# IQTLabs/WITW

Measured on AMD Instinct MI355X. Metric: image-pairs/sec (embedding+similarity), higher is better.
Workload: dtype f32

## Files before the change

witw_amd/csrc/conv3x3.hip:

```cpp
#include "common.h"
#include <stdlib.h>
#include <algorithm>

namespace {

constexpr int TW_WIDE = 64;

__device__ const f32x4 g_zero_f4[1] = {{0.f, 0.f, 0.f, 0.f}};

struct ConvArgs {
    const float* x;
    const float* wpk;
    const float* bias;
    const float* dropmask;
    const float* post_scale;
    const float* post_shift;
    float lrelu;
    unsigned char* pool_code;
    const float* gate;
    float* y;
    int B, H, W, Cin, Cout;
    int Ho, Wo;
    int tiles_x, tiles_y;
    int n_tiles, sp_total, sp_per_xcd, xcd_map;
    int circ, relu, out_nchw;
    int force_nw;
    int force_geo;
    int dil_h;
    int tap_base;
    int ksplit, kc_per_split;
    size_t split_stride;
    int s2d, s2d_h, s2d_w, valid_h, valid_w;
    int wino;
    const float* wpk_wino;
#ifdef WITW_STAMPS
    unsigned long long* stamps;
#endif
};

template <int NW, bool POOL>
__device__ __forceinline__ void conv_wino_h2(const ConvArgs& p, f32x4* smem) {
    constexpr int TH = NW, TW = 64, IW = TW + 2, IH = TH + 2;
    constexpr int NTHREADS = 64 * NW;
    constexpr int WTN = 64;
    constexpr int IN_F4 = 2 * IH * IW;
    constexpr int W_F4 = 12 * 2 * WTN;
    constexpr int STAGE_F4 = IN_F4 + W_F4;
    constexpr int NIN = (IN_F4 + NTHREADS - 1) / NTHREADS;
    constexpr int NWT = W_F4 / NTHREADS;
    static_assert(NWT * NTHREADS == W_F4, "the filter slab splits evenly over the workgroup");

    const int tid = threadIdx.x;
    const int lane = tid & 63;
    const int wave = tid >> 6;
    const int l31 = lane & 31;
    const int hq = lane >> 5;

    int ntile, sp;
    if (p.xcd_map) {
        const int g = blockIdx.x >> 3;
        ntile = g % p.n_tiles;
        sp = (blockIdx.x & 7) * p.sp_per_xcd + g / p.n_tiles;
        if (sp >= p.sp_total) return;
    } else {
        ntile = blockIdx.x / p.sp_total;
        sp = blockIdx.x - ntile * p.sp_total;
    }
    const int tiles_img = p.tiles_x * p.tiles_y;
    const int b = sp / tiles_img;
    sp -= b * tiles_img;
    const int ty = sp / p.tiles_x;
    const int tx = sp - ty * p.tiles_x;
    const int oy0 = ty * TH;
    const int ox0 = tx * TW;
    const int n0 = ntile * WTN;
    const int nkc = p.Cin >> 3;

    constexpr unsigned OOR = 0x80000000u;
    const size_t img_floats = (size_t)p.H * p.W * p.Cin;
    __amdgpu_buffer_rsrc_t in_rs = __builtin_amdgcn_make_buffer_rsrc((void*)(p.x + (size_t)b * img_floats), 0,
                                                                     (unsigned)(img_floats * 4), 0x00020000);
    __amdgpu_buffer_rsrc_t w_rs = __builtin_amdgcn_make_buffer_rsrc(
        (void*)(reinterpret_cast<const f32x4*>(p.wpk_wino) + (size_t)ntile * nkc * W_F4), 0, (unsigned)nkc * W_F4 * 16u, 0x00020000);
    unsigned gin[NIN];
#pragma unroll
    for (int i = 0; i < NIN; ++i) {
        const int s = tid + i * NTHREADS;
        const int pix = s >> 1, q = s & 1;
        const int r = pix / IW, c = pix - r * IW;
        const int gr = oy0 - 1 + r;
        int gc = ox0 - 1 + c;
        bool ok = (s < IN_F4) && gr >= 0 && gr < p.H;
        if (p.circ) {
            gc %= p.W;
            if (gc < 0) gc += p.W;
        } else {
            ok = ok && gc >= 0 && gc < p.W;
        }
        gin[i] = ok ? (unsigned)((((size_t)gr * p.W + gc) * p.Cin + q * 4) * 4) : OOR;
    }
    const unsigned gwoff = (unsigned)tid * 16u;
    f32x4 rin[NIN], rw[NWT];
    auto load_stage = [&](int kc) {
#pragma unroll
        for (int i = 0; i < NIN; ++i)
            rin[i] = __builtin_bit_cast(f32x4, __builtin_amdgcn_raw_buffer_load_b128(in_rs, gin[i], (unsigned)kc * 32u, 0));
        const unsigned wbase = (unsigned)kc * W_F4 * 16u;
#pragma unroll
        for (int i = 0; i < NWT; ++i)
            rw[i] = __builtin_bit_cast(f32x4, __builtin_amdgcn_raw_buffer_load_b128(w_rs, gwoff, wbase + (unsigned)i * (NTHREADS * 16u), 0));
    };
    auto store_stage = [&](int buf) {
        f32x4* in_s = smem + buf * STAGE_F4;
        f32x4* w_s = in_s + IN_F4;
#pragma unroll
        for (int i = 0; i < NIN; ++i) {
            const int s = tid + i * NTHREADS;
            f32x4* dst = (NIN * NTHREADS == IN_F4 || s < IN_F4) ? in_s + (s & 1) * (IH * IW) + (s >> 1) : smem + 2 * STAGE_F4;
            *dst = rin[i];
        }
#pragma unroll
        for (int i = 0; i < NWT; ++i) w_s[tid + i * NTHREADS] = rw[i];
    };

    const int wm = wave >> 1, wn = wave & 1;
    const int abase = hq * (IH * IW) + 2 * wm * IW + l31;
    const int wbase = hq * WTN + wn * 32 + l31;
    f32x16 acc[4][2];
#pragma unroll
    for (int t = 0; t < 4; ++t)
#pragma unroll
        for (int ct = 0; ct < 2; ++ct)
#pragma unroll
            for (int r = 0; r < 16; ++r) acc[t][ct][r] = 0.f;

    f32x4 fa[2][4], fb[2][4];
    auto read_a = [&](int set, const f32x4* in_s, int s) {
#pragma unroll
        for (int i = 0; i < 4; ++i) fa[set][i] = in_s[abase + i * IW + 32 * (s & 1) + (s >> 1)];
    };
    auto read_b = [&](int set, const f32x4* w_s, int kw) {
#pragma unroll
        for (int t = 0; t < 4; ++t) fb[set][t] = w_s[(kw * 4 + t) * 2 * WTN + wbase];
    };
    auto transform = [&](int set) {
#pragma unroll
        for (int j = 0; j < 4; ++j) {
            const float d0 = fa[set][0][j], d1 = fa[set][1][j], d2 = fa[set][2][j], d3 = fa[set][3][j];
            fa[set][0][j] = d0 - d2;
            fa[set][1][j] = d1 + d2;
            fa[set][2][j] = d2 - d1;
            fa[set][3][j] = d1 - d3;
        }
    };
    auto mfma_step = [&](int set, int bset, int ct) {
#pragma unroll
        for (int j = 0; j < 4; ++j)
#pragma unroll
            for (int t = 0; t < 4; ++t)
                acc[t][ct] = __builtin_amdgcn_mfma_f32_32x32x2f32(fa[set][t][j], fb[bset][t][j], acc[t][ct], 0, 0, 0);
    };

    load_stage(0);
    store_stage(0);
    __syncthreads();
    read_a(0, smem, 0);
    read_b(0, smem + IN_F4, 0);
    transform(0);

#define SG_STEP(NR, MASK, NX)                                           \
    do {                                                                \
        _Pragma("unroll") for (int i_ = 0; i_ < (NR); ++i_) {           \
            __builtin_amdgcn_sched_group_barrier(0x008, 1, 0);          \
            __builtin_amdgcn_sched_group_barrier(0x100, 1, 0);          \
        }                                                               \
        _Pragma("unroll") for (int i_ = 0; i_ < (NX); ++i_) {           \
            __builtin_amdgcn_sched_group_barrier(0x008, 1, 0);          \
            __builtin_amdgcn_sched_group_barrier(MASK, 1, 0);           \
        }                                                               \
        _Pragma("unroll") for (int i_ = 0; i_ < 16 - (NR) - (NX); ++i_) \
            __builtin_amdgcn_sched_group_barrier(0x008, 1, 0);          \
    } while (0)
    static_assert(16 - 4 - (NIN + NWT) >= 0, "step too short to hide the staging instructions");

    for (int kc = 0; kc < nkc; ++kc) {
        const int cur = kc & 1;
        const int kn = (kc + 1 < nkc) ? kc + 1 : kc;
        const f32x4* in_s = smem + cur * STAGE_F4;
        const f32x4* w_s = in_s + IN_F4;
        const f32x4* in_n = smem + (cur ^ 1) * STAGE_F4;
        read_a(1, in_s, 1);
        load_stage(kn);
        mfma_step(0, 0, 0);
        transform(1);
        SG_STEP(4, 0x020, NIN + NWT);
        read_a(0, in_s, 2);
        read_b(1, w_s, 1);
        mfma_step(1, 0, 1);
        transform(0);
        SG_STEP(8, 0x020, 0);
        read_a(1, in_s, 3);
        read_b(0, w_s, 2);
        mfma_step(0, 1, 0);
        transform(1);
        SG_STEP(8, 0x020, 0);
        read_a(0, in_s, 4);
        store_stage(cur ^ 1);
        mfma_step(1, 1, 1);
        transform(0);
        SG_STEP(4, 0x200, NIN + NWT);
        read_a(1, in_s, 5);
        mfma_step(0, 0, 0);
        transform(1);
        SG_STEP(4, 0x020, 0);
        __syncthreads();
        read_a(0, in_n, 0);
        read_b(1, in_n + IN_F4, 0);
        mfma_step(1, 0, 1);
        transform(0);
        SG_STEP(8, 0x020, 0);
#pragma unroll
        for (int t = 0; t < 4; ++t) fb[0][t] = fb[1][t];
    }
#undef SG_STEP

    f32x16 yv[2][2];
#pragma unroll
    for (int ct = 0; ct < 2; ++ct)
#pragma unroll
        for (int r = 0; r < 16; ++r) {
            const float m0 = acc[0][ct][r], m1 = acc[1][ct][r], m2 = acc[2][ct][r], m3 = acc[3][ct][r];
            yv[0][ct][r] = (m0 + m1) + m2;
            yv[1][ct][r] = (m1 - m2) - m3;
        }
    const int nb = n0 + wn * 32;
    const int nch = nb + l31;
    const float bv = p.bias[nch];
    const float dm = (p.dropmask != nullptr && nch < p.Cout) ? p.dropmask[(size_t)b * p.Cout + nch] : 1.f;
    const int act = p.relu;
    auto fin = [&](float v) {
        v = (v + bv) * dm;
        if (act == 1) v = fmaxf(v, 0.f);
        else if (act == 2) v = v > 0.f ? v : v * p.lrelu;
        return v;
    };
    const int Hy = POOL ? (p.Ho >> 1) : p.Ho;
    const int Wy = POOL ? (p.Wo >> 1) : p.Wo;
    float* slab = reinterpret_cast<float*>(smem) + wave * (32 * 32);
    const int prow = lane >> 3, pc4 = (lane & 7) * 4;
    if constexpr (!POOL) {
#pragma unroll
        for (int k = 0; k < 2; ++k)
#pragma unroll
            for (int ct = 0; ct < 2; ++ct) {
#pragma unroll
                for (int r = 0; r < 16; ++r) slab[((r & 3) + 8 * (r >> 2) + 4 * hq) * 32 + l31] = fin(yv[k][ct][r]);
                const int yy = oy0 + 2 * wm + k;
#pragma unroll
                for (int g = 0; g < 4; ++g) {
                    const int m = g * 8 + prow;
                    const f32x4 v = *reinterpret_cast<const f32x4*>(slab + m * 32 + pc4);
                    const int xx = ox0 + 32 * ct + m;
                    if (yy < Hy && xx < Wy && nb + pc4 < p.Cout)
                        __builtin_nontemporal_store(v, reinterpret_cast<f32x4*>(p.y + (((size_t)b * Hy + yy) * Wy + xx) * p.Cout + nb + pc4));
                }
            }
    } else {
        const int yy = (oy0 + 2 * wm) >> 1;
#pragma unroll
        for (int ct = 0; ct < 2; ++ct)
#pragma unroll
            for (int g = 0; g < 4; ++g)
#pragma unroll
                for (int e = 0; e < 2; ++e) {
                    const int r = 4 * g + 2 * e;
                    const float a00 = yv[0][ct][r], a01 = yv[0][ct][r + 1], a10 = yv[1][ct][r], a11 = yv[1][ct][r + 1];
                    const float m = fmaxf(fmaxf(a00, a01), fmaxf(a10, a11));
                    const int pc = 16 * ct + 4 * g + 2 * hq + e;
                    slab[pc * 32 + l31] = fin(m);
                    const int xx = (ox0 >> 1) + pc;
                    if (p.pool_code != nullptr && yy < Hy && xx < Wy && nch < p.Cout) {
                        const int code = (a00 == m) ? 0 : (a01 == m) ? 1 : (a10 == m) ? 2 : 3;
                        p.pool_code[(((size_t)b * Hy + yy) * Wy + xx) * p.Cout + nch] = (unsigned char)code;
                    }
                }
#pragma unroll
        for (int g = 0; g < 4; ++g) {
            const int pc = g * 8 + prow;
            const f32x4 v = *reinterpret_cast<const f32x4*>(slab + pc * 32 + pc4);
            const int xx = (ox0 >> 1) + pc;
            if (yy < Hy && xx < Wy && nb + pc4 < p.Cout)
                __builtin_nontemporal_store(v, reinterpret_cast<f32x4*>(p.y + (((size_t)b * Hy + yy) * Wy + xx) * p.Cout + nb + pc4));
        }
    }
}

template <int TN, int SH, bool POOL, int NW, int GEO, int TAPS = 9>
__global__ __launch_bounds__(64 * NW) void conv3x3_nhwc_f32_kernel(ConvArgs p) {
    static_assert(TAPS == 9 || TAPS == 4, "3x3 window or a 2x2 sub-window");
    constexpr bool NARROW = GEO == 1;
    constexpr bool DIL = GEO == 2;
    static_assert(!DIL || (TN == 128 && NW == 8 && SH == 1 && TAPS == 9 && !POOL), "the dilated form exists for the 8-wave 128-channel tile");
    constexpr int TH = NARROW ? 4 * NW : NW;
    constexpr int TW = NARROW ? 16 : 64;
    constexpr int IW = TW + 2;
    constexpr int NTHREADS = 64 * NW;
    constexpr int IH = (TH - 1) * SH + 3;
    constexpr int IN_F4 = 2 * IH * IW;
    constexpr int W_F4 = TAPS * 2 * TN;
    constexpr int STAGE_F4 = IN_F4 + W_F4;
    constexpr int NIN = (IN_F4 + NTHREADS - 1) / NTHREADS;
    constexpr int NWT = (W_F4 + NTHREADS - 1) / NTHREADS;
    constexpr int WGM = (TN == 128) ? NW / 2 : NW;
    constexpr int WM = (2 * NW) / WGM;
    constexpr int WN = 2;

    constexpr bool WINO = SH == 1 && TAPS == 9 && GEO == 0 && (TN == 128 || POOL);
    constexpr int WINO_F4 = WINO ? 2 * (2 * (NW + 2) * IW + 12 * 2 * 64) + 1 : 0;
    constexpr int DIRECT_F4 = (2 * STAGE_F4 + 1 > NW * 512) ? 2 * STAGE_F4 + 1 : NW * 512;
    constexpr int SMEM_F4 = DIRECT_F4 > WINO_F4 ? DIRECT_F4 : WINO_F4;
    __shared__ f32x4 smem[SMEM_F4];
    static_assert(SMEM_F4 * 16 >= NW * 32 * 64 * 4, "the buffer must hold one epilogue slab per wave");
    if constexpr (WINO) {
        if (p.wino) {
            conv_wino_h2<NW, POOL>(p, smem);
            return;
        }
    }

    const int tid = threadIdx.x;
    const int lane = tid & 63;
    const int wave = tid >> 6;
    const int l31 = lane & 31;
    const int hq = lane >> 5;

    int ntile, sp;
    if (p.xcd_map) {
        const int g = blockIdx.x >> 3;
        ntile = g % p.n_tiles;
        sp = (blockIdx.x & 7) * p.sp_per_xcd + g / p.n_tiles;
        if (sp >= p.sp_total) return;
    } else {
        ntile = blockIdx.x / p.sp_total;
        sp = blockIdx.x - ntile * p.sp_total;
    }
    const int tiles_img = p.tiles_x * p.tiles_y;
    const int b = sp / tiles_img;
    sp -= b * tiles_img;
    const int ty = sp / p.tiles_x;
    const int tx = sp - ty * p.tiles_x;
    const int oy0 = ty * TH;
    const int ox0 = tx * TW;
    const int n0 = ntile * TN;
    int nkc = p.Cin >> 3;
    int kc_lo = 0;
    if constexpr (TAPS == 4) {
        if (p.ksplit > 1) {
            kc_lo = (int)blockIdx.y * p.kc_per_split;
            nkc = min(nkc - kc_lo, p.kc_per_split);
        }
    }

    constexpr unsigned OOR = 0x80000000u;
    const int Hp = p.dil_h ? (p.H - 1) / 2 + 1 : p.H;
    const size_t img_floats = (size_t)Hp * p.W * p.Cin;
    __amdgpu_buffer_rsrc_t in_rs = __builtin_amdgcn_make_buffer_rsrc(
        (void*)(p.x + (size_t)b * img_floats + (size_t)kc_lo * 8), 0, (unsigned)(img_floats * 4) - (unsigned)kc_lo * 32u, 0x00020000);
    const unsigned wtile_bytes = (unsigned)nkc * W_F4 * 16u;
    __amdgpu_buffer_rsrc_t w_rs = __builtin_amdgcn_make_buffer_rsrc(
        (void*)(reinterpret_cast<const f32x4*>(p.wpk) + ((size_t)ntile * (p.Cin >> 3) + kc_lo) * W_F4), 0, wtile_bytes, 0x00020000);
    unsigned gin[NIN];
#pragma unroll
    for (int i = 0; i < NIN; ++i) {
        const int s = tid + i * NTHREADS;
        const int pix = s >> 1, q = s & 1;
        const int r = pix / IW, c = pix - r * IW;
        const int gr = oy0 * SH - 1 + r;
        int gc = ox0 - 1 + c;
        bool ok = (s < IN_F4) && gr >= 0 && gr < p.H;
        int grp = gr;
        if (p.dil_h) {
            ok = ok && (gr & 1) == 0;
            grp = gr >> 1;
        }
        if (p.circ) {
            gc %= p.W;
            if (gc < 0) gc += p.W;
        } else {
            ok = ok && gc >= 0 && gc < p.W;
        }
        gin[i] = ok ? (unsigned)((((size_t)grp * p.W + gc) * p.Cin + q * 4) * 4) : OOR;
    }
    const unsigned gwoff = (unsigned)tid * 16u;

    f32x4 rin[NIN], rw[NWT];
    auto load_stage = [&](int kc) {
#pragma unroll
        for (int i = 0; i < NIN; ++i)
            rin[i] = __builtin_bit_cast(f32x4, __builtin_amdgcn_raw_buffer_load_b128(in_rs, gin[i], (unsigned)kc * 32u, 0));
        const unsigned wbase = (unsigned)kc * W_F4 * 16u;
#pragma unroll
        for (int i = 0; i < NWT; ++i)
            rw[i] = __builtin_bit_cast(f32x4, __builtin_amdgcn_raw_buffer_load_b128(w_rs, gwoff, wbase + (unsigned)i * (NTHREADS * 16u), 0));
    };
    auto store_stage = [&](int buf) {
        f32x4* in_s = smem + buf * STAGE_F4;
        f32x4* w_s = in_s + IN_F4;
#pragma unroll
        for (int i = 0; i < NIN; ++i) {
            const int s = tid + i * NTHREADS;
            f32x4* dst = (NIN * NTHREADS == IN_F4 || s < IN_F4) ? in_s + (s & 1) * (IH * IW) + (s >> 1) : smem + 2 * STAGE_F4;
            *dst = rin[i];
        }
#pragma unroll
        for (int i = 0; i < NWT; ++i) {
            const int s = tid + i * NTHREADS;
            f32x4* dst = (NWT * NTHREADS == W_F4 || s < W_F4) ? w_s + s : smem + 2 * STAGE_F4;
            *dst = rw[i];
        }
    };

    const int wm = (TN == 128) ? (wave >> 1) : wave;
    const int wn = (TN == 128) ? (wave & 1) : 0;
    int trow[WM], tcol[WM];
#pragma unroll
    for (int mt = 0; mt < WM; ++mt) {
        if (NARROW) {
            trow[mt] = 2 * ((TN == 128 ? 4 : 2) * wm + mt);
            tcol[mt] = 0;
        } else if (TN == 128) {
            trow[mt] = 2 * wm + (mt >> 1);
            tcol[mt] = 32 * (mt & 1);
        } else {
            trow[mt] = 2 * (wm >> 1) + mt;
            tcol[mt] = 32 * (wm & 1);
        }
    }
    auto m_row = [](int m) { return NARROW ? (m >> 4) : 0; };
    auto m_col = [](int m) { return NARROW ? (m & 15) : m; };
    int abase[WM];
#pragma unroll
    for (int mt = 0; mt < WM; ++mt)
        abase[mt] = hq * (IH * IW) + (trow[mt] + m_row(l31)) * SH * IW + tcol[mt] + m_col(l31) + (TAPS == 4 ? p.tap_base * (IW + 1) : 0);
    const int wbase = hq * TN + wn * 64 + l31;

    f32x16 acc[WM][WN];
#pragma unroll
    for (int mt = 0; mt < WM; ++mt)
#pragma unroll
        for (int nt = 0; nt < WN; ++nt)
#pragma unroll
            for (int r = 0; r < 16; ++r) acc[mt][nt][r] = 0.f;

    f32x4 fa[2][WM], fb[2][WN];
    auto live = [](int mt, int tap) { return !DIL || ((((mt >> 1) + tap / 3) & 1) == 1); };
    auto read_frags = [&](int set, const f32x4* in_s, const f32x4* w_s, int tap) {
        const int kh = (TAPS == 4) ? (tap >> 1) : tap / 3, kw = (TAPS == 4) ? (tap & 1) : tap - kh * 3;
#pragma unroll
        for (int mt = 0; mt < WM; ++mt)
            if (live(mt, tap)) fa[set][mt] = in_s[abase[mt] + kh * IW + kw];
#pragma unroll
        for (int nt = 0; nt < WN; ++nt) fb[set][nt] = w_s[tap * 2 * TN + wbase + nt * 32];
    };
    auto mfma_tap = [&](int set, int tap) {
#pragma unroll
        for (int j = 0; j < 4; ++j)
#pragma unroll
            for (int mt = 0; mt < WM; ++mt)
                if (live(mt, tap)) {
#pragma unroll
                    for (int nt = 0; nt < WN; ++nt)
                        acc[mt][nt] =
                            __builtin_amdgcn_mfma_f32_32x32x2f32(fa[set][mt][j], fb[set][nt][j], acc[mt][nt], 0, 0, 0);
                }
    };

#ifdef WITW_STAMPS
    unsigned long long t_stamp[6];
    int n_stamp = 0;
#define STAMP() do { if (n_stamp < 6) t_stamp[n_stamp++] = __builtin_amdgcn_s_memtime(); } while (0)
    const unsigned long long r_stamp0 = __builtin_amdgcn_s_memrealtime();
#else
#define STAMP() do { } while (0)
#endif
    STAMP();
    load_stage(0);
    store_stage(0);
    __syncthreads();
    read_frags(0, smem, smem + IN_F4, 0);
    STAMP();

    constexpr int MPT = 4 * (DIL ? WM / 2 : WM) * WN;
    constexpr int RPT = (DIL ? WM / 2 : WM) + WN;
#define SG_PLAIN_TAP()                                                  \
    do {                                                                \
        _Pragma("unroll") for (int i_ = 0; i_ < RPT; ++i_) {            \
            __builtin_amdgcn_sched_group_barrier(0x008, 2, 0);          \
            __builtin_amdgcn_sched_group_barrier(0x100, 1, 0);          \
        }                                                               \
        _Pragma("unroll") for (int i_ = 0; i_ < MPT - 2 * RPT; ++i_)    \
            __builtin_amdgcn_sched_group_barrier(0x008, 1, 0);          \
    } while (0)
#define SG_HEAVY_TAP(MASK, NX)                                          \
    do {                                                                \
        _Pragma("unroll") for (int i_ = 0; i_ < RPT; ++i_) {            \
            __builtin_amdgcn_sched_group_barrier(0x008, 1, 0);          \
            __builtin_amdgcn_sched_group_barrier(0x100, 1, 0);          \
        }                                                               \
        _Pragma("unroll") for (int i_ = 0; i_ < (NX); ++i_) {           \
            __builtin_amdgcn_sched_group_barrier(0x008, 1, 0);          \
            __builtin_amdgcn_sched_group_barrier(MASK, 1, 0);           \
        }                                                               \
        _Pragma("unroll") for (int i_ = 0; i_ < MPT - RPT - (NX); ++i_) \
            __builtin_amdgcn_sched_group_barrier(0x008, 1, 0);          \
    } while (0)
    static_assert(MPT - RPT - (NIN + NWT) >= 0, "tap too short to hide the staging instructions");

    if constexpr (TAPS == 4) {
        for (int kc = 0; kc < nkc; ++kc) {
            const int cur = kc & 1;
            const int kn = (kc + 1 < nkc) ? kc + 1 : kc;
            const f32x4* in_s = smem + cur * STAGE_F4;
            const f32x4* w_s = in_s + IN_F4;
            const f32x4* in_n = smem + (cur ^ 1) * STAGE_F4;
            read_frags(1, in_s, w_s, 1);
            load_stage(kn);
            mfma_tap(0, 0);
            SG_HEAVY_TAP(0x020, NIN + NWT);
            read_frags(0, in_s, w_s, 2);
            mfma_tap(1, 1);
            SG_PLAIN_TAP();
            read_frags(1, in_s, w_s, 3);
            store_stage(cur ^ 1);
            mfma_tap(0, 2);
            SG_HEAVY_TAP(0x200, NIN + NWT);
            __syncthreads();
            read_frags(0, in_n, in_n + IN_F4, 0);
            mfma_tap(1, 3);
            SG_PLAIN_TAP();
        }
    } else {
        for (int kc = 0; kc < nkc; ++kc) {
            const int cur = kc & 1;
            const int kn = (kc + 1 < nkc) ? kc + 1 : kc;
            const f32x4* in_s = smem + cur * STAGE_F4;
            const f32x4* w_s = in_s + IN_F4;
            const f32x4* in_n = smem + (cur ^ 1) * STAGE_F4;
            read_frags(1, in_s, w_s, 1);
#ifndef WITW_DIAG_NOSTAGE
            load_stage(kn);
#endif
            mfma_tap(0, 0);
            SG_HEAVY_TAP(0x020, NIN + NWT);
#pragma unroll
            for (int tap = 1; tap < 4; ++tap) {
                read_frags((tap + 1) & 1, in_s, w_s, tap + 1);
                mfma_tap(tap & 1, tap);
                SG_PLAIN_TAP();
            }
            read_frags(1, in_s, w_s, 5);
#ifndef WITW_DIAG_NOSTAGE
            store_stage(cur ^ 1);
#endif
            mfma_tap(0, 4);
            SG_HEAVY_TAP(0x200, NIN + NWT);
#pragma unroll
            for (int tap = 5; tap < 8; ++tap) {
                read_frags((tap + 1) & 1, in_s, w_s, tap + 1);
                mfma_tap(tap & 1, tap);
                SG_PLAIN_TAP();
            }
#ifndef WITW_DIAG_NOBARRIER
            __syncthreads();
#endif
            read_frags(1, in_n, in_n + IN_F4, 0);
            mfma_tap(0, 8);
            SG_PLAIN_TAP();
#pragma unroll
            for (int mt = 0; mt < WM; ++mt) fa[0][mt] = fa[1][mt];
#pragma unroll
            for (int nt = 0; nt < WN; ++nt) fb[0][nt] = fb[1][nt];
        }
    }
#undef SG_PLAIN_TAP
#undef SG_HEAVY_TAP

    STAMP();
    float bv[WN], dm[WN], ps[WN], pt[WN];
    int nch[WN];
    int act = p.relu;
    bool has_post = p.post_scale != nullptr;
    bool raw = false;
    if constexpr (TAPS == 4) {
        raw = p.ksplit > 1;
        if (raw) { act = 0; has_post = false; }
    }
#pragma unroll
    for (int nt = 0; nt < WN; ++nt) {
        nch[nt] = n0 + wn * 64 + nt * 32 + l31;
        bv[nt] = raw ? 0.f : p.bias[nch[nt]];
        dm[nt] = 1.f;
        if (p.dropmask != nullptr && nch[nt] < p.Cout) dm[nt] = p.dropmask[(size_t)b * p.Cout + nch[nt]];
        ps[nt] = 1.f;
        pt[nt] = 0.f;
        if (has_post && nch[nt] < p.Cout) {
            ps[nt] = p.post_scale[nch[nt]];
            pt[nt] = p.post_shift[nch[nt]];
        }
    }
    auto fin = [&](float v, int nt) {
        v = (v + bv[nt]) * dm[nt];
        if (act == 1) v = fmaxf(v, 0.f);
        else if (act == 2) v = v > 0.f ? v : v * p.lrelu;
        if (has_post) v = v * ps[nt] + pt[nt];
        return v;
    };
    const int Hy = POOL ? (p.Ho >> 1) : p.Ho;
    const int Wy = POOL ? (p.Wo >> 1) : p.Wo;

    auto emit = [&](float v, int nt, int yy, int xx) {
        v = fin(v, nt);
        if (yy < Hy && xx < Wy && nch[nt] < p.Cout) {
            size_t o;
            if (p.out_nchw)
                o = (((size_t)b * p.Cout + nch[nt]) * Hy + yy) * Wy + xx;
            else
                o = (((size_t)b * Hy + yy) * Wy + xx) * p.Cout + nch[nt];
            if (p.gate != nullptr && !(p.gate[o] > 0.f)) v = 0.f;
            p.y[o] = v;
        }
    };

    if (!POOL && !p.out_nchw && (p.Cout & 3) == 0) {
        float* slab = reinterpret_cast<float*>(smem) + wave * (32 * 64);
        const int prow = lane >> 4, pc4 = (lane & 15) * 4;
#pragma unroll
        for (int mt = 0; mt < WM; ++mt) {
#pragma unroll
            for (int nt = 0; nt < WN; ++nt)
#pragma unroll
                for (int r = 0; r < 16; ++r) {
                    const float v = fin(acc[mt][nt][r], nt);
                    slab[((r & 3) + 8 * (r >> 2) + 4 * hq) * 64 + nt * 32 + l31] = v;
                }
            const int nbase = n0 + wn * 64 + pc4;
#pragma unroll
            for (int g = 0; g < 8; ++g) {
                const int m = g * 4 + prow;
                const f32x4 v = *reinterpret_cast<const f32x4*>(slab + m * 64 + pc4);
                const int yy = oy0 + trow[mt] + m_row(m);
                const int xx = ox0 + tcol[mt] + m_col(m);
                bool ok = yy < Hy && xx < Wy && nbase < p.Cout;
                size_t o = (((size_t)b * Hy + yy) * Wy + xx) * p.Cout + nbase;
                f32x4 w = v;
                if constexpr (TAPS == 4) {
                    if (p.ksplit > 1) {
                        o += (size_t)blockIdx.y * p.split_stride;
                    } else if (p.s2d) {
                        ok = yy < 2 * p.s2d_h && xx < 2 * p.s2d_w && nbase < p.Cout;
                        o = ((((size_t)b * p.s2d_h + (yy >> 1)) * p.s2d_w + (xx >> 1)) * 4 + (yy & 1) * 2 + (xx & 1)) * p.Cout + nbase;
                        if (!(yy < p.valid_h && xx < p.valid_w)) w = f32x4{0.f, 0.f, 0.f, 0.f};
                    }
                }
                if (ok) {
                    if (p.gate != nullptr) {
                        const f32x4 gt = *reinterpret_cast<const f32x4*>(p.gate + o);
#pragma unroll
                        for (int e = 0; e < 4; ++e) w[e] = gt[e] > 0.f ? v[e] : 0.f;
                    }
                    __builtin_nontemporal_store(w, reinterpret_cast<f32x4*>(p.y + o));
                }
            }
        }
    } else if (!POOL) {
#pragma unroll
        for (int mt = 0; mt < WM; ++mt)
#pragma unroll
            for (int nt = 0; nt < WN; ++nt)
#pragma unroll
                for (int r = 0; r < 16; ++r) {
                    const int m = (r & 3) + 8 * (r >> 2) + 4 * hq;
                    emit(acc[mt][nt][r], nt, oy0 + trow[mt] + m_row(m), ox0 + tcol[mt] + m_col(m));
                }
    } else if (NARROW) {
#pragma unroll
        for (int mt = 0; mt < WM; ++mt) {
            const int yy = (oy0 + trow[mt]) >> 1;
#pragma unroll
            for (int nt = 0; nt < WN; ++nt)
#pragma unroll
                for (int r = 0; r < 8; r += 2) {
                    const float a00 = acc[mt][nt][r], a01 = acc[mt][nt][r + 1];
                    const float a10 = acc[mt][nt][r + 8], a11 = acc[mt][nt][r + 9];
                    const float m = fmaxf(fmaxf(a00, a01), fmaxf(a10, a11));
                    const int xx = (ox0 >> 1) + (((r & 3) >> 1) | (hq << 1) | (((r >> 2) & 1) << 2));
                    emit(m, nt, yy, xx);
                    if (p.pool_code != nullptr && yy < Hy && xx < Wy && nch[nt] < p.Cout) {
                        const int code = (a00 == m) ? 0 : (a01 == m) ? 1 : (a10 == m) ? 2 : 3;
                        p.pool_code[(((size_t)b * Hy + yy) * Wy + xx) * p.Cout + nch[nt]] = (unsigned char)code;
                    }
                }
        }
    } else if ((p.Cout & 3) == 0 && p.gate == nullptr) {
        float* slab = reinterpret_cast<float*>(smem) + wave * (32 * 64);
        const int prow = lane >> 4, pc4 = (lane & 15) * 4;
#pragma unroll
        for (int pr = 0; pr < WM / 2; ++pr) {
            const int mtA = (TN == 128) ? (pr & 1) : 0;
            const int mtB = (TN == 128) ? (2 + (pr & 1)) : 1;
            const int yy = (oy0 + trow[mtA]) >> 1;
            const int xb = (ox0 + tcol[mtA]) >> 1;
#pragma unroll
            for (int nt = 0; nt < WN; ++nt)
#pragma unroll
                for (int g = 0; g < 4; ++g)
#pragma unroll
                    for (int e = 0; e < 2; ++e) {
                        const float a00 = acc[mtA][nt][4 * g + 2 * e], a01 = acc[mtA][nt][4 * g + 2 * e + 1];
                        const float a10 = acc[mtB][nt][4 * g + 2 * e], a11 = acc[mtB][nt][4 * g + 2 * e + 1];
                        const float m = fmaxf(fmaxf(a00, a01), fmaxf(a10, a11));
                        const int pc = 4 * g + 2 * hq + e;
                        slab[pc * 64 + nt * 32 + l31] = fin(m, nt);
                        if (p.pool_code != nullptr && yy < Hy && xb + pc < Wy && nch[nt] < p.Cout) {
                            const int code = (a00 == m) ? 0 : (a01 == m) ? 1 : (a10 == m) ? 2 : 3;
                            p.pool_code[(((size_t)b * Hy + yy) * Wy + xb + pc) * p.Cout + nch[nt]] = (unsigned char)code;
                        }
                    }
            const int nbase = n0 + wn * 64 + pc4;
#pragma unroll
            for (int g = 0; g < 4; ++g) {
                const int pc = g * 4 + prow;
                const f32x4 v = *reinterpret_cast<const f32x4*>(slab + pc * 64 + pc4);
                if (yy < Hy && xb + pc < Wy && nbase < p.Cout)
                    __builtin_nontemporal_store(v, reinterpret_cast<f32x4*>(p.y + (((size_t)b * Hy + yy) * Wy + xb + pc) * p.Cout + nbase));
            }
        }
    } else {
#pragma unroll
        for (int pr = 0; pr < WM / 2; ++pr) {
            const int mtA = (TN == 128) ? (pr & 1) : 0;
            const int mtB = (TN == 128) ? (2 + (pr & 1)) : 1;
#pragma unroll
            for (int nt = 0; nt < WN; ++nt)
#pragma unroll
                for (int g = 0; g < 4; ++g)
#pragma unroll
                    for (int e = 0; e < 2; ++e) {
                        const float a00 = acc[mtA][nt][4 * g + 2 * e], a01 = acc[mtA][nt][4 * g + 2 * e + 1];
                        const float a10 = acc[mtB][nt][4 * g + 2 * e], a11 = acc[mtB][nt][4 * g + 2 * e + 1];
                        const float v0 = fmaxf(a00, a01);
                        const float v1 = fmaxf(a10, a11);
                        const int yy = (oy0 + trow[mtA]) >> 1;
                        const int xx = ((ox0 + tcol[mtA]) >> 1) + 4 * g + 2 * hq + e;
                        emit(fmaxf(v0, v1), nt, yy, xx);
                        if (p.pool_code != nullptr && yy < Hy && xx < Wy && nch[nt] < p.Cout) {
                            const float m = fmaxf(v0, v1);
                            const int code = (a00 == m) ? 0 : (a01 == m) ? 1 : (a10 == m) ? 2 : 3;
                            p.pool_code[(((size_t)b * Hy + yy) * Wy + xx) * p.Cout + nch[nt]] = (unsigned char)code;
                        }
                    }
        }
    }
#ifdef WITW_STAMPS
    asm volatile("s_waitcnt vmcnt(0)" ::: "memory");
    STAMP();
    if (lane == 0 && p.stamps != nullptr) {
        unsigned long long* o = p.stamps + ((size_t)blockIdx.x * NW + wave) * 8;
        for (int i = 0; i < n_stamp; ++i) o[i] = t_stamp[i];
        o[6] = __builtin_amdgcn_s_memrealtime() - r_stamp0;
        o[7] = n_stamp;
    }
#endif
}

__global__ void pack_weights_kernel(const float* __restrict__ w, float* __restrict__ wpk, int Cout, int Cin,
                                    int n_tiles, int nkc, int TN, int transpose_flip, int src_cout, int src_cin, int taps,
                                    int tap_base) {
    const size_t total = (size_t)n_tiles * nkc * taps * 2 * TN;
    const size_t idx = (size_t)blockIdx.x * blockDim.x + threadIdx.x;
    if (idx >= total) return;
    size_t t = idx;
    const int n = t % TN; t /= TN;
    const int q = t % 2; t /= 2;
    const int tap = t % taps; t /= taps;
    const int kc = t % nkc; t /= nkc;
    const int nt = (int)t;
    const int kh = (taps == 4) ? tap_base + (tap >> 1) : tap / 3, kw = (taps == 4) ? tap_base + (tap & 1) : tap % 3;
    const int co = nt * TN + n;
    f32x4 v = {0.f, 0.f, 0.f, 0.f};
#pragma unroll
    for (int j = 0; j < 4; ++j) {
        const int ci = kc * 8 + q * 4 + j;
        if (co < Cout && ci < Cin) {
            if (!transpose_flip)
                v[j] = w[(((size_t)co * src_cin + ci) * 3 + kh) * 3 + kw];
            else
                v[j] = w[(((size_t)ci * src_cin + co) * 3 + (2 - kh)) * 3 + (2 - kw)];
        }
    }
    reinterpret_cast<f32x4*>(wpk)[idx] = v;
}

__global__ void pack_weights_wino_kernel(const float* __restrict__ w, float* __restrict__ wpk, int Cout, int Cin, int nkc,
                                         size_t total) {
    const size_t idx = (size_t)blockIdx.x * blockDim.x + threadIdx.x;
    if (idx >= total) return;
    size_t t = idx;
    const int n = t % 64; t /= 64;
    const int q = t % 2; t /= 2;
    const int tr = t % 4; t /= 4;
    const int kw = t % 3; t /= 3;
    const int kc = t % nkc; t /= nkc;
    const int co = (int)t * 64 + n;
    f32x4 v = {0.f, 0.f, 0.f, 0.f};
#pragma unroll
    for (int j = 0; j < 4; ++j) {
        const int ci = kc * 8 + q * 4 + j;
        if (co < Cout && ci < Cin) {
            const float* g = w + ((size_t)co * Cin + ci) * 9 + kw;
            const float g0 = g[0], g1 = g[3], g2 = g[6];
            v[j] = tr == 0 ? g0 : tr == 1 ? ((g0 + g1) + g2) * 0.5f : tr == 2 ? ((g0 - g1) + g2) * 0.5f : g2;
        }
    }
    reinterpret_cast<f32x4*>(wpk)[idx] = v;
}

__global__ void nchw_to_nhwc8_kernel(const float* __restrict__ x, float* __restrict__ y, int B, int C, int H, int W) {
    const size_t npix = (size_t)B * H * W;
    const size_t idx = (size_t)blockIdx.x * blockDim.x + threadIdx.x;
    if (idx >= npix) return;
    const size_t hw = (size_t)H * W;
    const size_t b = idx / hw, r = idx - b * hw;
    float v[8];
#pragma unroll
    for (int c = 0; c < 8; ++c) v[c] = (c < C) ? x[(b * C + c) * hw + r] : 0.f;
    f32x4* o = reinterpret_cast<f32x4*>(y + idx * 8);
    o[0] = f32x4{v[0], v[1], v[2], v[3]};
    o[1] = f32x4{v[4], v[5], v[6], v[7]};
}

__global__ void nchw_to_nhwc_kernel(const float* __restrict__ x, float* __restrict__ y, int C, int Cp, size_t hw, size_t total) {
    const size_t idx = (size_t)blockIdx.x * blockDim.x + threadIdx.x;
    if (idx >= total) return;
    const int c = idx % Cp;
    const size_t t = idx / Cp;
    const size_t b = t / hw, r = t - b * hw;
    y[idx] = (c < C) ? x[(b * C + c) * hw + r] : 0.f;
}

template <int TN, int SH, bool POOL, int NW, int GEO, int TAPS = 9>
int launch_conv_nw(ConvArgs a, hipStream_t st) {
    a.tiles_y = cdiv(a.Ho, GEO == 1 ? 4 * NW : NW);
    a.tiles_x = cdiv(a.Wo, GEO == 1 ? 16 : 64);
    const long long sp_total = (long long)a.B * a.tiles_x * a.tiles_y;
    a.n_tiles = cdiv(a.Cout, a.wino ? 64 : TN);
    a.sp_per_xcd = (int)((sp_total + 7) / 8);
    if (sp_total < 8) a.xcd_map = 0;
    const long long grid = a.xcd_map ? 8LL * a.sp_per_xcd * a.n_tiles : sp_total * a.n_tiles;
    if (grid <= 0 || grid > 0x7fffffffLL || sp_total > 0x7fffffffLL) {
        witw_set_error("conv3x3: grid %lld out of range", grid);
        return WITW_ERR_INVALID;
    }
    a.sp_total = (int)sp_total;
    const unsigned gy = (TAPS == 4 && a.ksplit > 1) ? (unsigned)a.ksplit : 1u;
    hipLaunchKernelGGL((conv3x3_nhwc_f32_kernel<TN, SH, POOL, NW, GEO, TAPS>), dim3((unsigned)grid, gy), dim3(64 * NW), 0, st, a);
    WITW_CHECK_LAUNCH("conv3x3_nhwc_f32");
    witw_note_variant("conv3x3_nhwc_f32_kernel<%d,%d,%s,%d,%d,%d>", TN, SH, POOL ? "true" : "false", NW, GEO, TAPS);
    if (a.wino) witw_note_conv_form("wino_h2");
    return WITW_OK;
}

int choose_waves(int B, int Ho, int Wo, int Cout, int force_nw) {
    const int TN = (Cout >= 128) ? 128 : 64;
    const long long big = (long long)cdiv(Cout, TN) * B * cdiv(Wo, TW_WIDE) * cdiv(Ho, 8);
    if (force_nw == 4) return 4;
    return (force_nw == 8 || ((Ho % 8) == 0 && witw_fills_rounds(big))) ? 8 : 4;
}

bool choose_narrow(int Wo, int force_geo) { return force_geo == 1 || (force_geo != 0 && Wo <= 32); }

int env_int(const char* name, int dflt) {
    const char* e = getenv(name);
    return e ? atoi(e) : dflt;
}

int g_dil_skip = -1;
int dil_skip() {
    if (g_dil_skip < 0) {
        const char* e = getenv("WITW_CONV_DILSKIP");
        g_dil_skip = e ? (atoi(e) != 0) : 1;
    }
    return g_dil_skip;
}

int g_wino = -1;
int wino_on() {
    if (g_wino < 0) {
        const char* e = getenv("WITW_CONV_WINO");
        g_wino = e ? (atoi(e) != 0) : 1;
    }
    return g_wino;
}

template <int TN, int SH, bool POOL>
int launch_conv(ConvArgs a, hipStream_t st) {
    const bool wino = SH == 1 && (TN == 128 || POOL) && a.wpk_wino != nullptr && wino_on() && a.gate == nullptr && !a.dil_h &&
                      !a.out_nchw && a.post_scale == nullptr && (a.Cout & 3) == 0 && a.force_geo != 1 &&
                      !choose_narrow(a.Wo, a.force_geo);
    a.wino = wino ? 1 : 0;
    if (wino) return choose_waves(a.B, a.Ho, a.Wo, a.Cout, a.force_nw) == 8 ? launch_conv_nw<TN, SH, POOL, 8, 0>(a, st)
                                                                          : launch_conv_nw<TN, SH, POOL, 4, 0>(a, st);
#ifndef WITW_NO_NARROW
    if (choose_narrow(a.Wo, a.force_geo)) return launch_conv_nw<TN, SH, POOL, 4, 1>(a, st);
#endif
    if (choose_waves(a.B, a.Ho, a.Wo, a.Cout, a.force_nw) == 8) {
        if constexpr (TN == 128 && SH == 1 && !POOL) {
            if (a.dil_h && dil_skip()) return launch_conv_nw<TN, SH, POOL, 8, 2>(a, st);
        }
        return launch_conv_nw<TN, SH, POOL, 8, 0>(a, st);
    }
    return launch_conv_nw<TN, SH, POOL, 4, 0>(a, st);
}

template <int TN>
int launch_conv_taps4(const ConvArgs& a, hipStream_t st) {
#ifndef WITW_NO_NARROW
    if (choose_narrow(a.Wo, a.force_geo)) return launch_conv_nw<TN, 1, false, 4, 1, 4>(a, st);
#endif
    if (choose_waves(a.B, a.Ho, a.Wo, a.Cout, a.force_nw) == 8) return launch_conv_nw<TN, 1, false, 8, 0, 4>(a, st);
    return launch_conv_nw<TN, 1, false, 4, 0, 4>(a, st);
}

}

#ifdef WITW_STAMPS
unsigned long long* witw_conv_stamps_ptr = nullptr;
#endif

extern "C" {

int witw_conv3x3_tile_n(int cout) { return cout >= 128 ? 128 : 64; }

int witw_conv3x3_workgroup_waves(int B, int H, int W, int Cout, int stride_h) {
    if (B <= 0 || H <= 0 || W <= 0 || Cout <= 0 || (stride_h != 1 && stride_h != 2)) return -1;
    if (choose_narrow(W, env_int("WITW_CONV_GEO", -1))) return 4;
    return choose_waves(B, (H + 2 - 3) / stride_h + 1, W, Cout, env_int("WITW_CONV_NW", 0));
}

long long witw_conv3x3_packed_floats(int cout, int cin) {
    if (cout <= 0 || cin <= 0) return -1;
    const int TN = witw_conv3x3_tile_n(cout);
    const long long n_tiles = cdiv(cout, TN), nkc = cdiv(cin, 8);
    return n_tiles * nkc * 9 * 2 * TN * 4;
}

int witw_conv3x3_bias_floats(int cout) {
    const int TN = witw_conv3x3_tile_n(cout);
    return cdiv(cout, TN) * TN;
}

int witw_conv3x3_pack_weights(const float* w_kcrs, float* wpk, int cout, int cin, int transpose_flip, void* stream) {
    WITW_CHECK_ARG(w_kcrs && wpk, "pack_weights: null pointer");
    WITW_CHECK_ARG(cout > 0 && cin > 0, "pack_weights: bad shape cout=%d cin=%d", cout, cin);
    const int TN = witw_conv3x3_tile_n(cout);
    const int n_tiles = cdiv(cout, TN), nkc = cdiv(cin, 8);
    const size_t total = (size_t)n_tiles * nkc * 9 * 2 * TN;
    const int src_cin = transpose_flip ? cout : cin;
    hipLaunchKernelGGL(pack_weights_kernel, dim3((unsigned)((total + 255) / 256)), dim3(256), 0, (hipStream_t)stream,
                       w_kcrs, wpk, cout, cin, n_tiles, nkc, TN, transpose_flip, cout, src_cin, 9, 0);
    WITW_CHECK_LAUNCH("pack_weights");
    return WITW_OK;
}

long long witw_conv3x3_packed_floats_taps4(int cout, int cin) {
    if (cout <= 0 || cin <= 0) return -1;
    const int TN = witw_conv3x3_tile_n(cout);
    return (long long)cdiv(cout, TN) * cdiv(cin, 8) * 4 * 2 * TN * 4;
}

int witw_conv3x3_pack_weights_taps4(const float* w_kcrs, float* wpk, int cout, int cin, int transpose_flip, void* stream) {
    WITW_CHECK_ARG(w_kcrs && wpk, "pack_weights_taps4: null pointer");
    WITW_CHECK_ARG(cout > 0 && cin > 0, "pack_weights_taps4: bad shape cout=%d cin=%d", cout, cin);
    const int TN = witw_conv3x3_tile_n(cout);
    const int n_tiles = cdiv(cout, TN), nkc = cdiv(cin, 8);
    const size_t total = (size_t)n_tiles * nkc * 4 * 2 * TN;
    const int src_cin = transpose_flip ? cout : cin;
    hipLaunchKernelGGL(pack_weights_kernel, dim3((unsigned)((total + 255) / 256)), dim3(256), 0, (hipStream_t)stream,
                       w_kcrs, wpk, cout, cin, n_tiles, nkc, TN, transpose_flip, cout, src_cin, 4, transpose_flip ? 0 : 1);
    WITW_CHECK_LAUNCH("pack_weights_taps4");
    return WITW_OK;
}

static long long taps4_workgroups(int B, int H, int W, int Cout) {
    const int TN = witw_conv3x3_tile_n(Cout);
    const long long nt = cdiv(Cout, TN);
    if (choose_narrow(W, env_int("WITW_CONV_GEO", -1))) return nt * B * cdiv(H, 16) * cdiv(W, 16);
    const int nw = choose_waves(B, H, W, Cout, env_int("WITW_CONV_NW", 0));
    return nt * B * cdiv(H, nw) * cdiv(W, 64);
}

int witw_conv3x3_taps4_ksplit(int B, int H, int W, int Cin, int Cout) {
    if (B <= 0 || H <= 0 || W <= 0 || Cin <= 0 || Cout <= 0) return -1;
    const int forced = env_int("WITW_CONV_KSPLIT", 0);
    const int nkc = Cin >> 3;
    const long long wg = taps4_workgroups(B, H, W, Cout);
    int S = 1;
    if (forced > 0) S = forced;
    else if (wg < 512 && nkc >= 64) {
        S = (int)std::min<long long>(32, (1024 + wg - 1) / wg);
        S = std::min(S, wg * (nkc / 32) >= 256 ? nkc / 32 : nkc / 8);
    }
    S = std::max(1, std::min(S, nkc));
    const int per = cdiv(nkc, S);
    return cdiv(nkc, per);
}

int witw_conv3x3_fwd_taps4_ex(const float* x, const float* wpk4, const float* bias, const float* gate, const float* post_scale,
                              const float* post_shift, float* y, int B, int H, int W, int Cin, int Cout, int relu,
                              float lrelu_slope, int tap_base, int ksplit, int s2d, int valid_h, int valid_w, void* stream) {
    WITW_CHECK_ARG(x && wpk4 && bias && y, "conv3x3_fwd_taps4: null pointer");
    WITW_CHECK_ARG(B > 0 && H > 0 && W > 0 && Cout > 0, "conv3x3_fwd_taps4: bad shape B=%d H=%d W=%d Cout=%d", B, H, W, Cout);
    WITW_CHECK_ARG(Cin > 0 && (Cin % 8) == 0, "conv3x3_fwd_taps4: Cin=%d must be a positive multiple of 8", Cin);
    WITW_CHECK_ARG(relu >= 0 && relu <= 2, "conv3x3_fwd_taps4: activation %d unknown (0 none, 1 ReLU, 2 LeakyReLU)", relu);
    WITW_CHECK_ARG(tap_base == 0 || tap_base == 1, "conv3x3_fwd_taps4: tap_base=%d outside {0,1}", tap_base);
    WITW_CHECK_ARG((post_scale == nullptr) == (post_shift == nullptr), "conv3x3_fwd_taps4: post_scale and post_shift go together");
    WITW_CHECK_ARG(ksplit >= 1 && ksplit <= 65535 && ksplit <= (Cin >> 3), "conv3x3_fwd_taps4: ksplit=%d outside [1, Cin/8]", ksplit);
    WITW_CHECK_ARG(!(ksplit > 1 && (gate || s2d)), "conv3x3_fwd_taps4: split-K writes raw partial sums (no gate, no s2d output)");
    WITW_CHECK_ARG(!((ksplit > 1 || s2d) && (Cout & 3)), "conv3x3_fwd_taps4: split-K / s2d output need Cout %% 4 == 0, got %d", Cout);
    WITW_CHECK_ARG(!(s2d && gate), "conv3x3_fwd_taps4: s2d output with gate unsupported");
    WITW_CHECK_ARG(!s2d || (valid_h > 0 && valid_w > 0 && valid_h <= H && valid_w <= W),
                   "conv3x3_fwd_taps4: valid region %dx%d outside the %dx%d map", valid_h, valid_w, H, W);
    WITW_CHECK_ARG(!s2d || (2 * ((valid_h + 1) / 2) <= H && 2 * ((valid_w + 1) / 2) <= W),
                   "conv3x3_fwd_taps4: s2d output of an odd valid size needs one more computed row / column");
    ConvArgs a;
    a.x = x; a.wpk = wpk4; a.bias = bias; a.dropmask = nullptr; a.gate = gate; a.y = y;
    a.post_scale = post_scale; a.post_shift = post_shift; a.lrelu = lrelu_slope;
    a.pool_code = nullptr;
    a.B = B; a.H = H; a.W = W; a.Cin = Cin; a.Cout = Cout;
    a.Ho = H; a.Wo = W;
    a.tiles_x = 0; a.tiles_y = 0;
    a.force_nw = env_int("WITW_CONV_NW", 0);
    a.force_geo = env_int("WITW_CONV_GEO", -1);
    a.xcd_map = env_int("WITW_CONV_XCD", 1) != 0;
    a.circ = 0; a.relu = relu; a.out_nchw = 0; a.dil_h = 0; a.tap_base = tap_base;
    a.ksplit = ksplit;
    a.wino = 0; a.wpk_wino = nullptr;
    a.kc_per_split = cdiv(Cin >> 3, ksplit);
    WITW_CHECK_ARG((long long)(ksplit - 1) * a.kc_per_split < (Cin >> 3), "conv3x3_fwd_taps4: ksplit=%d leaves an empty K slice", ksplit);
    a.split_stride = (size_t)B * H * W * Cout;
    a.s2d = s2d ? 1 : 0;
    a.valid_h = valid_h; a.valid_w = valid_w;
    a.s2d_h = (valid_h + 1) / 2; a.s2d_w = (valid_w + 1) / 2;
#ifdef WITW_STAMPS
    a.stamps = witw_conv_stamps_ptr;
#endif
    hipStream_t st = (hipStream_t)stream;
    return witw_conv3x3_tile_n(Cout) == 128 ? launch_conv_taps4<128>(a, st) : launch_conv_taps4<64>(a, st);
}

int witw_conv3x3_fwd_taps4(const float* x, const float* wpk4, const float* bias, const float* gate, const float* post_scale,
                           const float* post_shift, float* y, int B, int H, int W, int Cin, int Cout, int relu,
                           float lrelu_slope, int tap_base, void* stream) {
    return witw_conv3x3_fwd_taps4_ex(x, wpk4, bias, gate, post_scale, post_shift, y, B, H, W, Cin, Cout, relu, lrelu_slope,
                                     tap_base, 1, 0, 0, 0, stream);
}

int witw_nchw_to_nhwc8(const float* x, float* y, int B, int C, int H, int W, void* stream) {
    WITW_CHECK_ARG(x && y, "nchw_to_nhwc8: null pointer");
    WITW_CHECK_ARG(B > 0 && C > 0 && C <= 8 && H > 0 && W > 0, "nchw_to_nhwc8: bad shape B=%d C=%d H=%d W=%d", B, C, H, W);
    const size_t npix = (size_t)B * H * W;
    hipLaunchKernelGGL(nchw_to_nhwc8_kernel, dim3((unsigned)((npix + 255) / 256)), dim3(256), 0, (hipStream_t)stream, x, y,
                       B, C, H, W);
    WITW_CHECK_LAUNCH("nchw_to_nhwc8");
    return WITW_OK;
}

int witw_nchw_to_nhwc(const float* x, float* y, int B, int C, int H, int W, int Cpad, void* stream) {
    WITW_CHECK_ARG(x && y, "nchw_to_nhwc: null pointer");
    WITW_CHECK_ARG(B > 0 && C > 0 && H > 0 && W > 0 && Cpad >= C, "nchw_to_nhwc: bad shape");
    const size_t total = (size_t)B * H * W * Cpad;
    hipLaunchKernelGGL(nchw_to_nhwc_kernel, dim3((unsigned)((total + 255) / 256)), dim3(256), 0, (hipStream_t)stream, x, y, C,
                       Cpad, (size_t)H * W, total);
    WITW_CHECK_LAUNCH("nchw_to_nhwc");
    return WITW_OK;
}

}

namespace {

int conv3x3_fwd_any(const float* x, const float* wpk, const float* wpk_wino, const float* bias, const float* dropmask,
                    const float* gate, const float* post_scale, const float* post_shift, float* y, unsigned char* pool_code, int B,
                    int H, int W, int Cin, int Cout, int stride_h, int pad_circular, int relu, float lrelu_slope, int pool,
                    int out_nchw, int dilate_h, void* stream) {
    WITW_CHECK_ARG(x && wpk && bias && y, "conv3x3_fwd: null pointer");
    WITW_CHECK_ARG(B > 0 && H > 0 && W > 0 && Cout > 0, "conv3x3_fwd: bad shape B=%d H=%d W=%d Cout=%d", B, H, W, Cout);
    WITW_CHECK_ARG(Cin > 0 && (Cin % 8) == 0, "conv3x3_fwd: Cin=%d must be a positive multiple of 8", Cin);
    WITW_CHECK_ARG(stride_h == 1 || stride_h == 2, "conv3x3_fwd: stride_h=%d unsupported", stride_h);
    WITW_CHECK_ARG(!(pool && stride_h == 2), "conv3x3_fwd: pool with stride 2 unsupported");
    WITW_CHECK_ARG(!(pool && out_nchw), "conv3x3_fwd: pool with NCHW output unsupported");
    WITW_CHECK_ARG(!(pool && gate), "conv3x3_fwd: pool with gate unsupported");
    WITW_CHECK_ARG(!(dilate_h && stride_h == 2), "conv3x3_fwd: dilated input with stride 2 unsupported");
    WITW_CHECK_ARG(relu >= 0 && relu <= 2, "conv3x3_fwd: activation %d unknown (0 none, 1 ReLU, 2 LeakyReLU)", relu);
    WITW_CHECK_ARG((post_scale == nullptr) == (post_shift == nullptr), "conv3x3_fwd: post_scale and post_shift go together");
    WITW_CHECK_ARG(!(pool && relu == 2) && !(pool && post_scale), "conv3x3_fwd: pool needs a monotone epilogue (ReLU only)");
    ConvArgs a;
    a.x = x; a.wpk = wpk; a.bias = bias; a.dropmask = dropmask; a.gate = gate; a.y = y;
    a.post_scale = post_scale; a.post_shift = post_shift; a.lrelu = lrelu_slope;
    a.pool_code = pool ? pool_code : nullptr;
    a.B = B; a.H = H; a.W = W; a.Cin = Cin; a.Cout = Cout;
    a.Ho = (H + 2 - 3) / stride_h + 1;
    a.Wo = W;
    a.tiles_x = 0;
    a.tiles_y = 0;
    a.force_nw = env_int("WITW_CONV_NW", 0);
    a.force_geo = env_int("WITW_CONV_GEO", -1);
    a.xcd_map = env_int("WITW_CONV_XCD", 1) != 0;
    a.circ = pad_circular; a.relu = relu; a.out_nchw = out_nchw; a.dil_h = dilate_h; a.tap_base = 0;
    a.ksplit = 1; a.kc_per_split = 0; a.split_stride = 0; a.s2d = 0; a.s2d_h = a.s2d_w = a.valid_h = a.valid_w = 0;
    a.wino = 0; a.wpk_wino = wpk_wino;
#ifdef WITW_STAMPS
    a.stamps = witw_conv_stamps_ptr;
#endif
    hipStream_t st = (hipStream_t)stream;
    const int TN = witw_conv3x3_tile_n(Cout);
    if (TN == 128) {
        if (stride_h == 2) return launch_conv<128, 2, false>(a, st);
        return pool ? launch_conv<128, 1, true>(a, st) : launch_conv<128, 1, false>(a, st);
    }
    if (stride_h == 2) return launch_conv<64, 2, false>(a, st);
    return pool ? launch_conv<64, 1, true>(a, st) : launch_conv<64, 1, false>(a, st);
}

}

extern "C" {

int witw_conv3x3_fwd_ex(const float* x, const float* wpk, const float* bias, const float* dropmask, const float* gate,
                        const float* post_scale, const float* post_shift, float* y, unsigned char* pool_code, int B, int H,
                        int W, int Cin, int Cout, int stride_h, int pad_circular, int relu, float lrelu_slope, int pool,
                        int out_nchw, int dilate_h, void* stream) {
    return conv3x3_fwd_any(x, wpk, nullptr, bias, dropmask, gate, post_scale, post_shift, y, pool_code, B, H, W, Cin, Cout,
                           stride_h, pad_circular, relu, lrelu_slope, pool, out_nchw, dilate_h, stream);
}

int witw_conv3x3_fwd_wino(const float* x, const float* wpk, const float* wpk_wino, const float* bias, const float* dropmask,
                          const float* gate, const float* post_scale, const float* post_shift, float* y, unsigned char* pool_code,
                          int B, int H, int W, int Cin, int Cout, int stride_h, int pad_circular, int relu, float lrelu_slope,
                          int pool, int out_nchw, int dilate_h, void* stream) {
    WITW_CHECK_ARG(wpk_wino, "conv3x3_fwd_wino: null Winograd filter");
    return conv3x3_fwd_any(x, wpk, wpk_wino, bias, dropmask, gate, post_scale, post_shift, y, pool_code, B, H, W, Cin, Cout,
                           stride_h, pad_circular, relu, lrelu_slope, pool, out_nchw, dilate_h, stream);
}

int witw_conv3x3_wino(int enable) {
    const int prev = wino_on();
    if (enable >= 0) g_wino = enable != 0;
    return prev;
}

long long witw_conv3x3_packed_floats_wino(int cout, int cin) {
    if (cout <= 0 || cin <= 0) return -1;
    return (long long)cdiv(cout, 64) * cdiv(cin, 8) * 12 * 2 * 64 * 4;
}

int witw_conv3x3_pack_weights_wino(const float* w_kcrs, float* wpk_wino, int cout, int cin, void* stream) {
    WITW_CHECK_ARG(w_kcrs && wpk_wino, "pack_weights_wino: null pointer");
    WITW_CHECK_ARG(cout > 0 && cin > 0, "pack_weights_wino: bad shape cout=%d cin=%d", cout, cin);
    const int n_tiles = cdiv(cout, 64), nkc = cdiv(cin, 8);
    const size_t total = (size_t)n_tiles * nkc * 12 * 2 * 64;
    hipLaunchKernelGGL(pack_weights_wino_kernel, dim3((unsigned)((total + 255) / 256)), dim3(256), 0, (hipStream_t)stream,
                       w_kcrs, wpk_wino, cout, cin, nkc, total);
    WITW_CHECK_LAUNCH("pack_weights_wino");
    return WITW_OK;
}

int witw_conv3x3_dil_skip(int enable) {
    const int prev = dil_skip();
    if (enable >= 0) g_dil_skip = enable != 0;
    return prev;
}

int witw_conv3x3_fwd(const float* x, const float* wpk, const float* bias, const float* dropmask, float* y, int B, int H,
                     int W, int Cin, int Cout, int stride_h, int pad_circular, int relu, int pool, int out_nchw,
                     void* stream) {
    return witw_conv3x3_fwd_ex(x, wpk, bias, dropmask, nullptr, nullptr, nullptr, y, nullptr, B, H, W, Cin, Cout, stride_h,
                               pad_circular, relu ? 1 : 0, 0.f, pool, out_nchw, 0, stream);
}

}
```

Before: 2390.

## Hand-interleave MFMA, LDS reads, global staging and transforms with sched barriers

Replaces the sched_group_barrier hints with explicit per-instruction interleaving inside the Winograd conv3x3 main loop. Each MFMA is followed by at most one LDS read, global load or LDS store, plus half a transform, and a full sched_barrier after each slot pins that order. B-fragment reads are spread across two steps and the __syncthreads moves to the middle of a step. The aim is tighter overlap of memory latency with matrix work, at the cost of the compiler losing freedom to reorder and a risk of exposed stalls if the fixed order is wrong.

```diff
diff --git a/witw_amd/csrc/conv3x3.hip b/witw_amd/csrc/conv3x3.hip
--- a/witw_amd/csrc/conv3x3.hip
+++ b/witw_amd/csrc/conv3x3.hip
@@ -101,26 +101,20 @@
     }
     const unsigned gwoff = (unsigned)tid * 16u;
     f32x4 rin[NIN], rw[NWT];
-    auto load_stage = [&](int kc) {
-#pragma unroll
-        for (int i = 0; i < NIN; ++i)
-            rin[i] = __builtin_bit_cast(f32x4, __builtin_amdgcn_raw_buffer_load_b128(in_rs, gin[i], (unsigned)kc * 32u, 0));
-        const unsigned wbase = (unsigned)kc * W_F4 * 16u;
-#pragma unroll
-        for (int i = 0; i < NWT; ++i)
-            rw[i] = __builtin_bit_cast(f32x4, __builtin_amdgcn_raw_buffer_load_b128(w_rs, gwoff, wbase + (unsigned)i * (NTHREADS * 16u), 0));
+    auto load_one = [&](int kc, int i) {
+        if (i < NIN) rin[i] = __builtin_bit_cast(f32x4, __builtin_amdgcn_raw_buffer_load_b128(in_rs, gin[i], (unsigned)kc * 32u, 0));
+        else rw[i - NIN] = __builtin_bit_cast(f32x4, __builtin_amdgcn_raw_buffer_load_b128(
+                 w_rs, gwoff, (unsigned)kc * W_F4 * 16u + (unsigned)(i - NIN) * (NTHREADS * 16u), 0));
     };
-    auto store_stage = [&](int buf) {
+    auto store_one = [&](int buf, int i) {
         f32x4* in_s = smem + buf * STAGE_F4;
-        f32x4* w_s = in_s + IN_F4;
-#pragma unroll
-        for (int i = 0; i < NIN; ++i) {
+        if (i < NIN) {
             const int s = tid + i * NTHREADS;
             f32x4* dst = (NIN * NTHREADS == IN_F4 || s < IN_F4) ? in_s + (s & 1) * (IH * IW) + (s >> 1) : smem + 2 * STAGE_F4;
             *dst = rin[i];
-        }
-#pragma unroll
-        for (int i = 0; i < NWT; ++i) w_s[tid + i * NTHREADS] = rw[i];
+        } else {
+            in_s[IN_F4 + tid + (i - NIN) * NTHREADS] = rw[i - NIN];
+        }
     };
 
     const int wm = wave >> 1, wn = wave & 1;
@@ -135,53 +129,51 @@
             for (int r = 0; r < 16; ++r) acc[t][ct][r] = 0.f;
 
     f32x4 fa[2][4], fb[2][4];
-    auto read_a = [&](int set, const f32x4* in_s, int s) {
-#pragma unroll
-        for (int i = 0; i < 4; ++i) fa[set][i] = in_s[abase + i * IW + 32 * (s & 1) + (s >> 1)];
-    };
-    auto read_b = [&](int set, const f32x4* w_s, int kw) {
-#pragma unroll
-        for (int t = 0; t < 4; ++t) fb[set][t] = w_s[(kw * 4 + t) * 2 * WTN + wbase];
-    };
-    auto transform = [&](int set) {
-#pragma unroll
-        for (int j = 0; j < 4; ++j) {
-            const float d0 = fa[set][0][j], d1 = fa[set][1][j], d2 = fa[set][2][j], d3 = fa[set][3][j];
+    auto read_a = [&](int set, const f32x4* in_s, int s, int i) { fa[set][i] = in_s[abase + i * IW + 32 * (s & 1) + (s >> 1)]; };
+    auto read_b = [&](int set, const f32x4* w_s, int kw, int t) { fb[set][t] = w_s[(kw * 4 + t) * 2 * WTN + wbase]; };
+    auto transform2 = [&](int set, int k) {
+        const int j = k >> 1;
+        const float d0 = fa[set][0][j], d1 = fa[set][1][j], d2 = fa[set][2][j], d3 = fa[set][3][j];
+        if ((k & 1) == 0) {
             fa[set][0][j] = d0 - d2;
+            fa[set][3][j] = d1 - d3;
+        } else {
             fa[set][1][j] = d1 + d2;
             fa[set][2][j] = d2 - d1;
-            fa[set][3][j] = d1 - d3;
         }
     };
-    auto mfma_step = [&](int set, int bset, int ct) {
-#pragma unroll
-        for (int j = 0; j < 4; ++j)
-#pragma unroll
-            for (int t = 0; t < 4; ++t)
-                acc[t][ct] = __builtin_amdgcn_mfma_f32_32x32x2f32(fa[set][t][j], fb[bset][t][j], acc[t][ct], 0, 0, 0);
+    auto mfma_one = [&](int set, int bset, int ct, int i) {
+        const int j = i >> 2, t = i & 3;
+        acc[t][ct] = __builtin_amdgcn_mfma_f32_32x32x2f32(fa[set][t][j], fb[bset][t][j], acc[t][ct], 0, 0, 0);
     };
 
-    load_stage(0);
-    store_stage(0);
+#pragma unroll
+    for (int i = 0; i < NIN + NWT; ++i) load_one(0, i);
+#pragma unroll
+    for (int i = 0; i < NIN + NWT; ++i) store_one(0, i);
     __syncthreads();
-    read_a(0, smem, 0);
-    read_b(0, smem + IN_F4, 0);
-    transform(0);
-
-#define SG_STEP(NR, MASK, NX)                                           \
-    do {                                                                \
-        _Pragma("unroll") for (int i_ = 0; i_ < (NR); ++i_) {           \
-            __builtin_amdgcn_sched_group_barrier(0x008, 1, 0);          \
-            __builtin_amdgcn_sched_group_barrier(0x100, 1, 0);          \
-        }                                                               \
-        _Pragma("unroll") for (int i_ = 0; i_ < (NX); ++i_) {           \
-            __builtin_amdgcn_sched_group_barrier(0x008, 1, 0);          \
-            __builtin_amdgcn_sched_group_barrier(MASK, 1, 0);           \
-        }                                                               \
-        _Pragma("unroll") for (int i_ = 0; i_ < 16 - (NR) - (NX); ++i_) \
-            __builtin_amdgcn_sched_group_barrier(0x008, 1, 0);          \
-    } while (0)
-    static_assert(16 - 4 - (NIN + NWT) >= 0, "step too short to hide the staging instructions");
+#pragma unroll
+    for (int i = 0; i < 4; ++i) read_b(0, smem + IN_F4, 0, i);
+    __builtin_amdgcn_sched_barrier(0);
+#pragma unroll
+    for (int i = 0; i < 4; ++i) read_a(0, smem, 0, i);
+#pragma unroll
+    for (int k = 0; k < 8; ++k) transform2(0, k);
+
+    auto step = [&](int set, int bset, int ct, auto&& mem, bool barrier_mid) {
+#pragma unroll
+        for (int i = 0; i < 16; ++i) {
+            mfma_one(set, bset, ct, i);
+            mem(i);
+            if (i >= 8) transform2(set ^ 1, i - 8);
+            __builtin_amdgcn_sched_barrier(0);
+            if (barrier_mid && i == 7) {
+                __syncthreads();
+                __builtin_amdgcn_sched_barrier(0);
+            }
+        }
+    };
+    static_assert(16 - 6 - (NIN + NWT) >= 0, "step too short to hide the staging instructions");
 
     for (int kc = 0; kc < nkc; ++kc) {
         const int cur = kc & 1;
@@ -189,40 +181,33 @@
         const f32x4* in_s = smem + cur * STAGE_F4;
         const f32x4* w_s = in_s + IN_F4;
         const f32x4* in_n = smem + (cur ^ 1) * STAGE_F4;
-        read_a(1, in_s, 1);
-        load_stage(kn);
-        mfma_step(0, 0, 0);
-        transform(1);
-        SG_STEP(4, 0x020, NIN + NWT);
-        read_a(0, in_s, 2);
-        read_b(1, w_s, 1);
-        mfma_step(1, 0, 1);
-        transform(0);
-        SG_STEP(8, 0x020, 0);
-        read_a(1, in_s, 3);
-        read_b(0, w_s, 2);
-        mfma_step(0, 1, 0);
-        transform(1);
-        SG_STEP(8, 0x020, 0);
-        read_a(0, in_s, 4);
-        store_stage(cur ^ 1);
-        mfma_step(1, 1, 1);
-        transform(0);
-        SG_STEP(4, 0x200, NIN + NWT);
-        read_a(1, in_s, 5);
-        mfma_step(0, 0, 0);
-        transform(1);
-        SG_STEP(4, 0x020, 0);
-        __syncthreads();
-        read_a(0, in_n, 0);
-        read_b(1, in_n + IN_F4, 0);
-        mfma_step(1, 0, 1);
-        transform(0);
-        SG_STEP(8, 0x020, 0);
+        step(0, 0, 0, [&](int i) {
+            if (i < 4) read_a(1, in_s, 1, i);
+            else if (i < 6) read_b(1, w_s, 1, i - 4);
+            else if (i < 6 + NIN + NWT) load_one(kn, i - 6);
+        }, false);
+        step(1, 0, 1, [&](int i) {
+            if (i < 4) read_a(0, in_s, 2, i);
+            else if (i < 6) read_b(1, w_s, 1, i - 2);
+        }, false);
+        step(0, 1, 0, [&](int i) {
+            if (i < 4) read_a(1, in_s, 3, i);
+            else if (i < 8) read_b(0, w_s, 2, i - 4);
+        }, false);
+        step(1, 1, 1, [&](int i) {
+            if (i < 4) read_a(0, in_s, 4, i);
+            else if (i < 4 + NIN + NWT) store_one(cur ^ 1, i - 4);
+        }, false);
+        step(0, 0, 0, [&](int i) {
+            if (i < 4) read_a(1, in_s, 5, i);
+        }, true);
+        step(1, 0, 1, [&](int i) {
+            if (i < 4) read_a(0, in_n, 0, i);
+            else if (i < 8) read_b(1, in_n + IN_F4, 0, i - 4);
+        }, false);
 #pragma unroll
         for (int t = 0; t < 4; ++t) fb[0][t] = fb[1][t];
     }
-#undef SG_STEP
 
     f32x16 yv[2][2];
 #pragma unroll
```

Measured after the change: 2496, median of 6. 4.4% higher.
